# PathologyFoundation/plip

Measured on NVIDIA H100. Metric: image-text pairs/sec (224x224, 77-tok), higher is better.
Workload: dtype bf16

## Files before the change

### plip_b200/csrc/attention.cu

```cuda
#include <cfloat>

#include "kernels.cuh"
#include "wgmma.cuh"

namespace plip {

namespace {

constexpr int kAttThreads = 256;
constexpr uint32_t kTileBytes = 128 * 64 * 2;
constexpr uint32_t kStageBytes = 3 * kTileBytes;
constexpr uint32_t kAttSmem = kStageBytes + 1024 + 64;

__device__ __forceinline__ float fast_exp2(float x) {
  float y;
  asm("ex2.approx.ftz.f32 %0, %1;" : "=f"(y) : "f"(x));
  return y;
}
constexpr float kLog2e = 1.4426950408889634f;


template <bool F16, int NK>
__device__ __forceinline__ void qk_scores(float (&s)[NK / 2], uint64_t qdesc, uint64_t kdesc) {
  wgmma_pin(s);
  wgmma_fence();
#pragma unroll
  for (int k = 0; k < kHeadDim / 16; ++k) {
    if constexpr (NK == 64) wgmma_ss_n64<F16>(s, qdesc + 2 * k, kdesc + 2 * k, k != 0 ? 1u : 0u);
    else wgmma_ss_n128<F16>(s, qdesc + 2 * k, kdesc + 2 * k, k != 0 ? 1u : 0u);
  }
  wgmma_commit();
  wgmma_wait<0>();
  wgmma_pin(s);
}

__device__ __forceinline__ void quad_max(float& a, float& b) {
#pragma unroll
  for (int o = 1; o < 4; o <<= 1) {
    a = fmaxf(a, __shfl_xor_sync(0xffffffffu, a, o));
    b = fmaxf(b, __shfl_xor_sync(0xffffffffu, b, o));
  }
}
__device__ __forceinline__ void quad_sum(float& a, float& b) {
#pragma unroll
  for (int o = 1; o < 4; o <<= 1) {
    a += __shfl_xor_sync(0xffffffffu, a, o);
    b += __shfl_xor_sync(0xffffffffu, b, o);
  }
}

__device__ __forceinline__ int last_visible_key(int row, int S, int causal) {
  return row < S ? (causal ? row : S - 1) : -1;
}

template <int N>
__device__ __forceinline__ void mask_column(float (&s)[N], int j, int e, bool ok, int key, int lim0, int lim1) {
  if (!(ok && key <= lim0)) s[4 * j + e] = -INFINITY;
  if (!(ok && key <= lim1)) s[4 * j + 2 + e] = -INFINITY;
}

__device__ __forceinline__ float row_shift(float m) { return fmaxf(m * kLog2e, -FLT_MAX); }
__device__ __forceinline__ float row_inv(float l) { return l > 0.f ? 1.0f / l : 0.f; }

__device__ __forceinline__ float softmax_exp(float s, float ms) { return fast_exp2(fmaf(s, kLog2e, -ms)); }

__device__ __forceinline__ float2 fold_row_max(const float (&s)[32], float& m0, float& m1, float& l0, float& l1) {
  float mx0 = m0, mx1 = m1;
#pragma unroll
  for (int j = 0; j < 8; ++j) {
    mx0 = fmaxf(mx0, fmaxf(s[4 * j + 0], s[4 * j + 1]));
    mx1 = fmaxf(mx1, fmaxf(s[4 * j + 2], s[4 * j + 3]));
  }
  quad_max(mx0, mx1);
  const float alpha0 = softmax_exp(m0, row_shift(mx0)), alpha1 = softmax_exp(m1, row_shift(mx1));
  m0 = mx0;
  m1 = mx1;
  l0 *= alpha0;
  l1 *= alpha1;
  return make_float2(alpha0, alpha1);
}

template <bool F16, int N>
__device__ __forceinline__ void exp_sum_pack(const float (&s)[N], float ms0, float ms1, float& l0, float& l1,
                                             uint32_t (&pa)[N / 8][4]) {
#pragma unroll
  for (int j = 0; j < N / 4; ++j) {
    const float e00 = softmax_exp(s[4 * j + 0], ms0), e01 = softmax_exp(s[4 * j + 1], ms0);
    const float e10 = softmax_exp(s[4 * j + 2], ms1), e11 = softmax_exp(s[4 * j + 3], ms1);
    l0 += e00 + e01;
    l1 += e10 + e11;
    pa[j >> 1][2 * (j & 1) + 0] = pack_op2<F16>(e00, e01);
    pa[j >> 1][2 * (j & 1) + 1] = pack_op2<F16>(e10, e11);
  }
}

template <bool F16>
__device__ __forceinline__ void stage_rows(uint32_t row0, const float (&o)[32], float inv0, float inv1, int rr, int q4) {
  const uint32_t row1 = row0 + 8u * 128u;
#pragma unroll
  for (int j = 0; j < 8; ++j) {
    st_shared_b32(row0 + ((j ^ rr) << 4) + q4 * 4, pack_op2<F16>(o[4 * j + 0] * inv0, o[4 * j + 1] * inv0));
    st_shared_b32(row1 + ((j ^ rr) << 4) + q4 * 4, pack_op2<F16>(o[4 * j + 2] * inv1, o[4 * j + 3] * inv1));
  }
}

struct AttParams {
  int64_t n_seq;
  int seq_len;
  int slot;
  int group;
  int heads;
  int64_t seq_tiles;
  int causal;
  const int32_t* key_mask;
};

template <bool F16, int NK>
__global__ void __launch_bounds__(kAttThreads, NK == 64 ? 3 : 2)
attention_kernel(const __grid_constant__ CUtensorMap tmLoad, const __grid_constant__ CUtensorMap tmStore,
                 const AttParams p) {
  extern __shared__ uint8_t smem_raw[];
  const uint32_t smem_base = (smem_u32(smem_raw) + 1023u) & ~1023u;
  const uint32_t bar = smem_base + kStageBytes;
  const uint32_t sq = smem_base, sk = smem_base + kTileBytes, sv = smem_base + 2 * kTileBytes;

  const int warp = threadIdx.x >> 5;
  const int lane = threadIdx.x & 31;
  const int hf = warp >> 2;
  const int D = p.heads * kHeadDim;
  const int S = p.seq_len, G = p.group, slot = p.slot;

  if (threadIdx.x == 0) {
    tma_prefetch_desc(&tmLoad);
    tma_prefetch_desc(&tmStore);
    mbar_init(bar, 1);
    fence_mbar_init();
  }
  __syncthreads();

  const int ntiles = (int)(p.seq_tiles * p.heads);
  const uint32_t slot_bytes = static_cast<uint32_t>(slot) * 128u;
  auto issue_loads = [&](int tile) {
    const int64_t st = tile / p.heads;
    const int h = (int)(tile - st * p.heads);
    mbar_arrive_expect_tx(bar, 3 * kTileBytes);
    for (int g = 0; g < G; ++g) {
      const int32_t row = (int32_t)((st * G + g) * S);
      tma_load_2d(sq + g * slot_bytes, &tmLoad, bar, h * kHeadDim, row);
      tma_load_2d(sk + g * slot_bytes, &tmLoad, bar, D + h * kHeadDim, row);
      tma_load_2d(sv + g * slot_bytes, &tmLoad, bar, 2 * D + h * kHeadDim, row);
    }
  };
  if (threadIdx.x == 0 && (int)blockIdx.x < ntiles) issue_loads(blockIdx.x);

  const int q4 = lane & 3, rr = lane >> 2;
  const int R0 = 64 * hf + 16 * (warp & 3) + rr;
  const int g = R0 / slot;
  const int r_in0 = R0 - g * slot, r_in1 = r_in0 + 8;
  const int kbase = (NK == 64) ? 64 * hf : 0;
  const int k_in_base = kbase - g * slot + 2 * q4;
  const int lim0 = last_visible_key(r_in0, S, p.causal), lim1 = last_visible_key(r_in1, S, p.causal);

  uint32_t it = 0;
  for (int tile = blockIdx.x; tile < ntiles; tile += gridDim.x, ++it) {
    const int st = tile / p.heads;
    const int h = tile - st * p.heads;
    const int64_t seq = (int64_t)st * G + g;

    uint32_t kv = 0;
#pragma unroll
    for (int c = 0; c < NK / 4; ++c) {
      const int k_in = k_in_base + 8 * (c >> 1) + (c & 1);
      bool ok = k_in >= 0 && k_in < S;
      if (ok && p.key_mask != nullptr) ok = seq < p.n_seq && p.key_mask[seq * S + k_in] != 0;
      kv |= (ok ? 1u : 0u) << c;
    }

    mbar_wait(bar, it & 1u);

    float s[NK / 2];
    qk_scores<F16, NK>(s, make_smem_desc_sw128(sq + hf * (64 * 128), 1024, 16),
                       make_smem_desc_sw128(sk + kbase * 128, 1024, 16));

    float mx0 = -INFINITY, mx1 = -INFINITY;
#pragma unroll
    for (int c = 0; c < NK / 4; ++c) {
      const int j = c >> 1, e = c & 1;
      mask_column(s, j, e, (kv >> c) & 1u, k_in_base + 8 * j + e, lim0, lim1);
      mx0 = fmaxf(mx0, s[4 * j + e]);
      mx1 = fmaxf(mx1, s[4 * j + 2 + e]);
    }
    quad_max(mx0, mx1);
    float sum0 = 0.f, sum1 = 0.f;
    uint32_t pa[NK / 16][4];
    exp_sum_pack<F16>(s, row_shift(mx0), row_shift(mx1), sum0, sum1, pa);
    quad_sum(sum0, sum1);

    float o[32];
    wgmma_pin(o);
    wgmma_fence();
#pragma unroll
    for (int kk = 0; kk < NK / 16; ++kk) {
      const uint64_t vdesc = make_smem_desc_sw128(sv + (kbase + 16 * kk) * 128, 1024, 1024);
      wgmma_rs_n64<F16>(o, pa[kk], vdesc, kk != 0 ? 1u : 0u);
    }
    wgmma_commit();
    wgmma_wait<0>();
    wgmma_pin(o);

    stage_rows<F16>(sq + static_cast<uint32_t>(R0) * 128u, o, row_inv(sum0), row_inv(sum1), rr, q4);
    fence_proxy_async_smem();
    __syncthreads();
    if (threadIdx.x == 0) {
      for (int gg = 0; gg < G; ++gg) {
        const int64_t sq_idx = (int64_t)st * G + gg;
        if (sq_idx < p.n_seq)
          tma_store_2d(&tmStore, sq + static_cast<uint32_t>(gg * slot) * 128u, h * kHeadDim, (int32_t)(sq_idx * S));
      }
      tma_store_commit();
      tma_store_wait_read();
      if (tile + (int)gridDim.x < ntiles) issue_loads(tile + gridDim.x);
    }
  }
  if (threadIdx.x == 0) tma_store_wait_all();
}

template <bool F16, int NK>
int launch_attention_inst(const CUtensorMap& tmL, const CUtensorMap& tmS, const AttParams& p, cudaStream_t st) {
  auto kern = attention_kernel<F16, NK>;
  static unsigned long long configured = 0;
  static int grid_cap = 0;
  if (first_use_on_device(configured)) {
    PLIP_CUDA_CHECK(cudaFuncSetAttribute(kern, cudaFuncAttributeMaxDynamicSharedMemorySize, (int)kAttSmem));
    int dev = 0, sms = 0, per_sm = 0;
    PLIP_CUDA_CHECK(cudaGetDevice(&dev));
    PLIP_CUDA_CHECK(cudaDeviceGetAttribute(&sms, cudaDevAttrMultiProcessorCount, dev));
    PLIP_CUDA_CHECK(cudaOccupancyMaxActiveBlocksPerMultiprocessor(&per_sm, kern, kAttThreads, kAttSmem));
    grid_cap = (per_sm > 0 ? per_sm : 1) * sms;
  }
  const int64_t tiles = p.seq_tiles * p.heads;
  const int grid = (int)(tiles < grid_cap ? tiles : grid_cap);
  PLIP_CUDA_CHECK(launch_kernel(kern, dim3(grid), dim3(kAttThreads), kAttSmem, st, 1, tmL, tmS, p));
  return 0;
}

constexpr int kLongThreads = 288;
constexpr int kLongKeys = 64;
constexpr uint32_t kLongQBytes = 128 * 64 * 2;
constexpr uint32_t kLongKVBytes = kLongKeys * 64 * 2;
constexpr int kLongStages = 2;
constexpr uint32_t kLongSmem = kLongQBytes + kLongStages * 2 * kLongKVBytes + 1024 + 64;

struct LongAttParams {
  int seq_len;
  int heads;
  int q_blocks;
};

template <bool F16>
__global__ void __launch_bounds__(kLongThreads, 2)
attention_long_kernel(const __grid_constant__ CUtensorMap tmQKV, const __grid_constant__ CUtensorMap tmO,
                      const LongAttParams p) {
  extern __shared__ uint8_t smem_raw[];
  const uint32_t smem_base = (smem_u32(smem_raw) + 1023u) & ~1023u;
  const uint32_t sq = smem_base;
  auto sk = [&](int s) { return smem_base + kLongQBytes + (uint32_t)s * 2u * kLongKVBytes; };
  auto sv = [&](int s) { return sk(s) + kLongKVBytes; };
  const uint32_t bar = smem_base + kLongQBytes + kLongStages * 2 * kLongKVBytes;
  const uint32_t q_bar = bar;
  auto full_bar = [&](int s) { return bar + 8u * (1 + s); };
  auto empty_bar = [&](int s) { return bar + 8u * (1 + kLongStages + s); };

  const int warp = threadIdx.x >> 5;
  const int lane = threadIdx.x & 31;
  const int wg = warp >> 2;
  const int S = p.seq_len, D = p.heads * kHeadDim;
  const int qb = blockIdx.x % p.q_blocks;
  const int bh = blockIdx.x / p.q_blocks;
  const int h = bh % p.heads;
  const int seq = bh / p.heads;
  const int q0 = qb * 128;
  const int n_kb = (S + kLongKeys - 1) / kLongKeys;

  if (threadIdx.x == 0) {
    tma_prefetch_desc(&tmQKV);
    tma_prefetch_desc(&tmO);
    mbar_init(q_bar, 1);
    for (int s = 0; s < kLongStages; ++s) {
      mbar_init(full_bar(s), 1);
      mbar_init(empty_bar(s), 2);
    }
    fence_mbar_init();
  }
  __syncthreads();

  if (wg == 2) {
    if (lane == 0) {
      mbar_arrive_expect_tx(q_bar, kLongQBytes);
      tma_load_3d(sq, &tmQKV, q_bar, h * kHeadDim, q0, seq);
      tma_load_3d(sq + kLongQBytes / 2, &tmQKV, q_bar, h * kHeadDim, q0 + 64, seq);
      for (int kb = 0; kb < n_kb; ++kb) {
        const int s = kb % kLongStages;
        if (kb >= kLongStages) mbar_wait(empty_bar(s), (uint32_t)((kb / kLongStages - 1) & 1));
        mbar_arrive_expect_tx(full_bar(s), 2 * kLongKVBytes);
        tma_load_3d(sk(s), &tmQKV, full_bar(s), D + h * kHeadDim, kb * kLongKeys, seq);
        tma_load_3d(sv(s), &tmQKV, full_bar(s), 2 * D + h * kHeadDim, kb * kLongKeys, seq);
      }
    }
    return;
  }

  const int q4 = lane & 3, rr = lane >> 2;
  const int R0 = 64 * wg + 16 * (warp & 3) + rr;
  float o[32];
#pragma unroll
  for (int i = 0; i < 32; ++i) o[i] = 0.f;
  float m0 = -INFINITY, m1 = -INFINITY;
  float l0 = 0.f, l1 = 0.f;
  const uint64_t qdesc = make_smem_desc_sw128(sq + wg * (64 * 128), 1024, 16);
  mbar_wait(q_bar, 0);

  for (int kb = 0; kb < n_kb; ++kb) {
    const int s = kb % kLongStages;
    mbar_wait(full_bar(s), (uint32_t)((kb / kLongStages) & 1));

    float sc[32];
    qk_scores<F16, 64>(sc, qdesc, make_smem_desc_sw128(sk(s), 1024, 16));

    const int kbase = kb * kLongKeys + 2 * q4;
    if (kb * kLongKeys + kLongKeys > S) {
#pragma unroll
      for (int j = 0; j < 8; ++j)
#pragma unroll
        for (int e = 0; e < 2; ++e)
          if (kbase + 8 * j + e >= S) {
            sc[4 * j + e] = -INFINITY;
            sc[4 * j + 2 + e] = -INFINITY;
          }
    }
    const float2 alpha = fold_row_max(sc, m0, m1, l0, l1);
#pragma unroll
    for (int j = 0; j < 8; ++j) {
      o[4 * j + 0] *= alpha.x; o[4 * j + 1] *= alpha.x;
      o[4 * j + 2] *= alpha.y; o[4 * j + 3] *= alpha.y;
    }
    uint32_t pa[4][4];
    exp_sum_pack<F16>(sc, row_shift(m0), row_shift(m1), l0, l1, pa);

    wgmma_pin(o);
    wgmma_fence();
#pragma unroll
    for (int kk = 0; kk < kLongKeys / 16; ++kk) {
      const uint64_t vdesc = make_smem_desc_sw128(sv(s) + 16 * kk * 128, 1024, 1024);
      wgmma_rs_n64<F16>(o, pa[kk], vdesc, 1u);
    }
    wgmma_commit();
    wgmma_wait<0>();
    wgmma_pin(o);
    if ((threadIdx.x & 127) == 0) mbar_arrive(empty_bar(s));
  }

  quad_sum(l0, l1);
  stage_rows<F16>(sq + static_cast<uint32_t>(R0) * 128u, o, row_inv(l0), row_inv(l1), rr, q4);
  fence_proxy_async_smem();
  if (wg == 0) named_barrier_sync<1, 128>();
  else named_barrier_sync<2, 128>();
  if ((threadIdx.x & 127) == 0 && q0 + 64 * wg < S) {
    tma_store_3d(&tmO, sq + wg * (64 * 128), h * kHeadDim, q0 + 64 * wg, seq);
    tma_store_commit();
    tma_store_wait_all();
  }
}

constexpr int kProbThreads = 128;
constexpr int kProbStages = 2;
constexpr int kProbLd = 72;
constexpr uint32_t kProbTileBytes = 64 * 64 * 2;
constexpr uint32_t kProbStageOff = kProbTileBytes;
constexpr uint32_t kProbStagingOff = kProbStageOff + kProbStages * kProbTileBytes;
constexpr uint32_t kProbBarOff = kProbStagingOff + 64 * kProbLd * 4;
constexpr uint32_t kProbSmem = kProbBarOff + 8 * (1 + kProbStages) + 1024;

struct ProbParams {
  int seq_len;
  int heads;
  int q_blocks;
  int causal;
  const int32_t* key_mask;
  float* probs;
};

template <bool F16>
__global__ void __launch_bounds__(kProbThreads)
attention_probs_kernel(const __grid_constant__ CUtensorMap tmQKV, const ProbParams p) {
  extern __shared__ uint8_t smem_raw[];
  const uint32_t smem_base = (smem_u32(smem_raw) + 1023u) & ~1023u;
  float* staging = reinterpret_cast<float*>(smem_raw + (smem_base - smem_u32(smem_raw)) + kProbStagingOff);
  const uint32_t sq = smem_base;
  auto sk = [&](int s) { return smem_base + kProbStageOff + (uint32_t)s * kProbTileBytes; };
  const uint32_t q_bar = smem_base + kProbBarOff;
  auto full_bar = [&](int s) { return q_bar + 8u * (1 + s); };

  const int warp = threadIdx.x >> 5;
  const int lane = threadIdx.x & 31;
  const int S = p.seq_len, D = p.heads * kHeadDim;
  const int qb = blockIdx.x % p.q_blocks;
  const int64_t bh = blockIdx.x / p.q_blocks;
  const int h = (int)(bh % p.heads);
  const int64_t seq = bh / p.heads;
  const int q0 = qb * 64;
  const int n_kb = (S + 63) / 64;
  const bool resident = n_kb <= kProbStages;
  const int n_loads = resident ? n_kb : 2 * n_kb;

  auto issue_k = [&](int i) {
    const int s = i % kProbStages;
    mbar_arrive_expect_tx(full_bar(s), kProbTileBytes);
    tma_load_3d(sk(s), &tmQKV, full_bar(s), D + h * kHeadDim, (i % n_kb) * 64, (int32_t)seq);
  };
  if (threadIdx.x == 0) {
    tma_prefetch_desc(&tmQKV);
    mbar_init(q_bar, 1);
    for (int s = 0; s < kProbStages; ++s) mbar_init(full_bar(s), 1);
    fence_mbar_init();
    mbar_arrive_expect_tx(q_bar, kProbTileBytes);
    tma_load_3d(sq, &tmQKV, q_bar, h * kHeadDim, q0, (int32_t)seq);
    for (int i = 0; i < kProbStages && i < n_loads; ++i) issue_k(i);
  }
  __syncthreads();

  const int q4 = lane & 3, rr = lane >> 2;
  const int r0 = 16 * warp + rr;
  const int qa = q0 + r0, qc = qa + 8;
  const int lim0 = last_visible_key(qa, S, p.causal), lim1 = last_visible_key(qc, S, p.causal);
  const int32_t* km = p.key_mask ? p.key_mask + seq * S : nullptr;
  const uint64_t qdesc = make_smem_desc_sw128(sq, 1024, 16);
  mbar_wait(q_bar, 0);

  float sc[32];
  auto scores = [&](int u) {
    const int li = resident ? u % n_kb : u;
    const int s = li % kProbStages;
    mbar_wait(full_bar(s), (uint32_t)((li / kProbStages) & 1));
    qk_scores<F16, 64>(sc, qdesc, make_smem_desc_sw128(sk(s), 1024, 16));
    if (!resident) {
      __syncthreads();
      if (threadIdx.x == 0 && li + kProbStages < n_loads) issue_k(li + kProbStages);
    }
    const int kbase = (u % n_kb) * 64 + 2 * q4;
#pragma unroll
    for (int j = 0; j < 8; ++j)
#pragma unroll
      for (int e = 0; e < 2; ++e) {
        const int key = kbase + 8 * j + e;
        mask_column(sc, j, e, key < S && (km == nullptr || km[key] != 0), key, lim0, lim1);
      }
  };

  float m0 = -INFINITY, m1 = -INFINITY, l0 = 0.f, l1 = 0.f;
  for (int kb = 0; kb < n_kb; ++kb) {
    scores(kb);
    fold_row_max(sc, m0, m1, l0, l1);
    const float ms0 = row_shift(m0), ms1 = row_shift(m1);
#pragma unroll
    for (int j = 0; j < 8; ++j) {
      l0 += softmax_exp(sc[4 * j + 0], ms0) + softmax_exp(sc[4 * j + 1], ms0);
      l1 += softmax_exp(sc[4 * j + 2], ms1) + softmax_exp(sc[4 * j + 3], ms1);
    }
  }
  quad_sum(l0, l1);
  const float ms0 = row_shift(m0), ms1 = row_shift(m1);
  const float inv0 = row_inv(l0), inv1 = row_inv(l1);

  float* wst = staging + 16 * warp * kProbLd;
  const int rows = S - (q0 + 16 * warp) < 16 ? S - (q0 + 16 * warp) : 16;
  float* out_base = p.probs + ((seq * p.heads + h) * (int64_t)S + q0 + 16 * warp) * S;
  for (int kb = 0; kb < n_kb; ++kb) {
    scores(n_kb + kb);
#pragma unroll
    for (int j = 0; j < 8; ++j) {
      *reinterpret_cast<float2*>(wst + rr * kProbLd + 8 * j + 2 * q4) =
          make_float2(softmax_exp(sc[4 * j + 0], ms0) * inv0, softmax_exp(sc[4 * j + 1], ms0) * inv0);
      *reinterpret_cast<float2*>(wst + (rr + 8) * kProbLd + 8 * j + 2 * q4) =
          make_float2(softmax_exp(sc[4 * j + 2], ms1) * inv1, softmax_exp(sc[4 * j + 3], ms1) * inv1);
    }
    __syncwarp();
    const int k0 = kb * 64;
    const int nc = S - k0 < 64 ? S - k0 : 64;
    const int total = rows > 0 ? rows * nc : 0;
    int r = 0, c = lane;
    while (c >= nc) { c -= nc; ++r; }
    for (int i = lane; i < total; i += 32) {
      __stcs(out_base + (int64_t)r * S + k0 + c, wst[r * kProbLd + c]);
      c += 32;
      while (c >= nc) { c -= nc; ++r; }
    }
    __syncwarp();
  }
}

template <auto Kern, int Threads, uint32_t Smem, typename... Args>
int launch_blocks(int64_t blocks, cudaStream_t st, const Args&... args) {
  static unsigned long long configured = 0;
  if (first_use_on_device(configured))
    PLIP_CUDA_CHECK(cudaFuncSetAttribute(Kern, cudaFuncAttributeMaxDynamicSharedMemorySize, (int)Smem));
  PLIP_CUDA_CHECK(launch_kernel(Kern, dim3((unsigned)blocks), dim3(Threads), Smem, st, 1, args...));
  return 0;
}

int check_attention_args(const char* fn, const void* qkv, const void* out, int64_t n_seq, int seq_len, int heads) {
  PLIP_REQUIRE(qkv && out, "%s: null argument", fn);
  PLIP_REQUIRE(n_seq > 0 && seq_len > 0 && seq_len <= kMaxVisSeq, "%s: bad shape n_seq=%lld seq_len=%d", fn,
               (long long)n_seq, seq_len);
  PLIP_REQUIRE(heads > 0 && heads <= 16, "%s: bad head count %d", fn, heads);
  return 0;
}

int make_seq_tmap(CUtensorMap* tm, const void* base, int64_t n_seq, int seq_len, int cols) {
  return make_tmap_bf16_3d(tm, base, (uint64_t)n_seq, (uint64_t)seq_len, (uint64_t)cols, (uint64_t)cols * 2,
                           (uint64_t)seq_len * cols * 2, 64, 64);
}

}

int launch_attention(const __nv_bfloat16* qkv, int64_t n_seq, int seq_len, int heads, bool causal,
                     const int32_t* key_mask, __nv_bfloat16* out, int f16, cudaStream_t st) {
  if (int rc = check_attention_args("attention", qkv, out, n_seq, seq_len, heads)) return rc;
  const int D = heads * kHeadDim;
  if (seq_len > 128) {
    PLIP_REQUIRE(!causal && key_mask == nullptr,
                 "attention: seq_len %d > 128 is supported without causal or key mask only", seq_len);
    LongAttParams p;
    p.seq_len = seq_len;
    p.heads = heads;
    p.q_blocks = (seq_len + 127) / 128;
    const int64_t blocks = n_seq * heads * p.q_blocks;
    PLIP_REQUIRE(blocks < 0x7fffffff && n_seq < 0x7fffffff, "attention: too many sequences");
    CUtensorMap tmQKV, tmO;
    if (int rc = make_seq_tmap(&tmQKV, qkv, n_seq, seq_len, 3 * D)) return rc;
    if (int rc = make_seq_tmap(&tmO, out, n_seq, seq_len, D)) return rc;
    return f16 ? launch_blocks<attention_long_kernel<true>, kLongThreads, kLongSmem>(blocks, st, tmQKV, tmO, p)
               : launch_blocks<attention_long_kernel<false>, kLongThreads, kLongSmem>(blocks, st, tmQKV, tmO, p);
  }
  const int64_t rows = n_seq * seq_len;
  PLIP_REQUIRE(rows + 128 < 0x7fffffff, "attention: too many token rows");
  AttParams p;
  p.n_seq = n_seq;
  p.seq_len = seq_len;
  p.slot = seq_len <= 32 ? 32 : (seq_len <= 64 ? 64 : 128);
  p.group = 128 / p.slot;
  p.heads = heads;
  p.seq_tiles = (n_seq + p.group - 1) / p.group;
  p.causal = causal ? 1 : 0;
  p.key_mask = key_mask;
  CUtensorMap tmL, tmS;
  if (int rc = make_tmap_bf16_2d(&tmL, qkv, (uint64_t)rows, (uint64_t)3 * D, (uint64_t)3 * D * 2, (uint32_t)p.slot, 64)) return rc;
  if (int rc = make_tmap_bf16_2d(&tmS, out, (uint64_t)rows, (uint64_t)D, (uint64_t)D * 2, (uint32_t)seq_len, 64)) return rc;
  PLIP_REQUIRE(p.seq_tiles * heads < 0x7fffffff, "attention: too many tiles");
  if (p.slot == 128) return f16 ? launch_attention_inst<true, 128>(tmL, tmS, p, st) : launch_attention_inst<false, 128>(tmL, tmS, p, st);
  return f16 ? launch_attention_inst<true, 64>(tmL, tmS, p, st) : launch_attention_inst<false, 64>(tmL, tmS, p, st);
}

int launch_attention_probs(const __nv_bfloat16* qkv, int64_t n_seq, int seq_len, int heads, bool causal,
                           const int32_t* key_mask, float* probs, int f16, cudaStream_t st) {
  if (int rc = check_attention_args("attention_probs", qkv, probs, n_seq, seq_len, heads)) return rc;
  ProbParams p;
  p.seq_len = seq_len;
  p.heads = heads;
  p.q_blocks = (seq_len + 63) / 64;
  p.causal = causal ? 1 : 0;
  p.key_mask = key_mask;
  p.probs = probs;
  const int64_t blocks = n_seq * heads * p.q_blocks;
  PLIP_REQUIRE(blocks < 0x7fffffff && n_seq < 0x7fffffff, "attention_probs: too many sequences");
  const int D = heads * kHeadDim;
  CUtensorMap tm;
  if (int rc = make_seq_tmap(&tm, qkv, n_seq, seq_len, 3 * D)) return rc;
  return f16 ? launch_blocks<attention_probs_kernel<true>, kProbThreads, kProbSmem>(blocks, st, tm, p)
             : launch_blocks<attention_probs_kernel<false>, kProbThreads, kProbSmem>(blocks, st, tm, p);
}

}
```

Measured before the change: 26970.

## Double-buffer attention tiles, skip dead rows, shorten causal chains, use 3D TMA loads

For the 128-key variant the attention kernel now keeps two shared-memory stages with separate mbarriers, so the loads for the next tile overlap compute on the current one. Warps whose rows fall past the sequence length skip the softmax and the output staging. Under a causal mask, the first warpgroup runs only 64 keys instead of 128. Q/K/V loads switch to a 3D tensor map indexed per sequence, so rows past a short sequence are zero-filled rather than read from the next sequence. In exchange, the NK=128 path uses double the shared memory, which may reduce occupancy, and the code adds a branchy helper template.

```diff
diff --git a/plip_b200/csrc/attention.cu b/plip_b200/csrc/attention.cu
--- a/plip_b200/csrc/attention.cu
+++ b/plip_b200/csrc/attention.cu
@@ -10,7 +10,6 @@
 constexpr int kAttThreads = 256;
 constexpr uint32_t kTileBytes = 128 * 64 * 2;
 constexpr uint32_t kStageBytes = 3 * kTileBytes;
-constexpr uint32_t kAttSmem = kStageBytes + 1024 + 64;
 
 __device__ __forceinline__ float fast_exp2(float x) {
   float y;
@@ -115,14 +114,58 @@
   const int32_t* key_mask;
 };
 
+template <bool F16, int NKW>
+__device__ __forceinline__ void attend_rows(uint32_t sq, uint32_t sk, uint32_t sv, int hf, int kbase, int k_in_base,
+                                            uint32_t kv, int lim0, int lim1, bool live, int R0, int rr, int q4) {
+  float s[NKW / 2];
+  qk_scores<F16, NKW>(s, make_smem_desc_sw128(sq + hf * (64 * 128), 1024, 16),
+                      make_smem_desc_sw128(sk + kbase * 128, 1024, 16));
+
+  float sum0 = 0.f, sum1 = 0.f;
+  uint32_t pa[NKW / 16][4] = {};
+  if (live) {
+    float mx0 = -INFINITY, mx1 = -INFINITY;
+#pragma unroll
+    for (int c = 0; c < NKW / 4; ++c) {
+      const int j = c >> 1, e = c & 1;
+      mask_column(s, j, e, (kv >> c) & 1u, k_in_base + 8 * j + e, lim0, lim1);
+      mx0 = fmaxf(mx0, s[4 * j + e]);
+      mx1 = fmaxf(mx1, s[4 * j + 2 + e]);
+    }
+    quad_max(mx0, mx1);
+    exp_sum_pack<F16>(s, row_shift(mx0), row_shift(mx1), sum0, sum1, pa);
+    quad_sum(sum0, sum1);
+  }
+
+  float o[32];
+  wgmma_pin(o);
+  wgmma_fence();
+#pragma unroll
+  for (int kk = 0; kk < NKW / 16; ++kk) {
+    const uint64_t vdesc = make_smem_desc_sw128(sv + (kbase + 16 * kk) * 128, 1024, 1024);
+    wgmma_rs_n64<F16>(o, pa[kk], vdesc, kk != 0 ? 1u : 0u);
+  }
+  wgmma_commit();
+  wgmma_wait<0>();
+  wgmma_pin(o);
+
+  if (live) stage_rows<F16>(sq + static_cast<uint32_t>(R0) * 128u, o, row_inv(sum0), row_inv(sum1), rr, q4);
+}
+
+template <int NK>
+constexpr int kAttStages = NK == 128 ? 2 : 1;
+template <int NK>
+constexpr uint32_t kAttSmem = kAttStages<NK> * kStageBytes + 1024 + 64;
+
 template <bool F16, int NK>
 __global__ void __launch_bounds__(kAttThreads, NK == 64 ? 3 : 2)
 attention_kernel(const __grid_constant__ CUtensorMap tmLoad, const __grid_constant__ CUtensorMap tmStore,
                  const AttParams p) {
+  constexpr int kStages = kAttStages<NK>;
   extern __shared__ uint8_t smem_raw[];
   const uint32_t smem_base = (smem_u32(smem_raw) + 1023u) & ~1023u;
-  const uint32_t bar = smem_base + kStageBytes;
-  const uint32_t sq = smem_base, sk = smem_base + kTileBytes, sv = smem_base + 2 * kTileBytes;
+  const uint32_t bar0 = smem_base + kStages * kStageBytes;
+  auto sq = [&](int s) { return smem_base + (uint32_t)s * kStageBytes; };
 
   const int warp = threadIdx.x >> 5;
   const int lane = threadIdx.x & 31;
@@ -133,39 +176,46 @@
   if (threadIdx.x == 0) {
     tma_prefetch_desc(&tmLoad);
     tma_prefetch_desc(&tmStore);
-    mbar_init(bar, 1);
+    for (int s = 0; s < kStages; ++s) mbar_init(bar0 + 8u * s, 1);
     fence_mbar_init();
   }
   __syncthreads();
 
   const int ntiles = (int)(p.seq_tiles * p.heads);
   const uint32_t slot_bytes = static_cast<uint32_t>(slot) * 128u;
-  auto issue_loads = [&](int tile) {
+  auto issue_loads = [&](int tile, int s) {
     const int64_t st = tile / p.heads;
     const int h = (int)(tile - st * p.heads);
+    const uint32_t bar = bar0 + 8u * s;
     mbar_arrive_expect_tx(bar, 3 * kTileBytes);
     for (int g = 0; g < G; ++g) {
-      const int32_t row = (int32_t)((st * G + g) * S);
-      tma_load_2d(sq + g * slot_bytes, &tmLoad, bar, h * kHeadDim, row);
-      tma_load_2d(sk + g * slot_bytes, &tmLoad, bar, D + h * kHeadDim, row);
-      tma_load_2d(sv + g * slot_bytes, &tmLoad, bar, 2 * D + h * kHeadDim, row);
+      const int32_t seq = (int32_t)(st * G + g);
+      const uint32_t dst = sq(s) + g * slot_bytes;
+      tma_load_3d(dst, &tmLoad, bar, h * kHeadDim, 0, seq);
+      tma_load_3d(dst + kTileBytes, &tmLoad, bar, D + h * kHeadDim, 0, seq);
+      tma_load_3d(dst + 2 * kTileBytes, &tmLoad, bar, 2 * D + h * kHeadDim, 0, seq);
     }
   };
-  if (threadIdx.x == 0 && (int)blockIdx.x < ntiles) issue_loads(blockIdx.x);
+  if (threadIdx.x == 0)
+    for (int s = 0; s < kStages; ++s)
+      if ((int)blockIdx.x + s * (int)gridDim.x < ntiles) issue_loads(blockIdx.x + s * gridDim.x, s);
 
   const int q4 = lane & 3, rr = lane >> 2;
   const int R0 = 64 * hf + 16 * (warp & 3) + rr;
   const int g = R0 / slot;
   const int r_in0 = R0 - g * slot, r_in1 = r_in0 + 8;
+  const bool live = r_in0 - rr < S;
   const int kbase = (NK == 64) ? 64 * hf : 0;
   const int k_in_base = kbase - g * slot + 2 * q4;
   const int lim0 = last_visible_key(r_in0, S, p.causal), lim1 = last_visible_key(r_in1, S, p.causal);
+  const bool short_chain = NK == 128 && p.causal && hf == 0;
 
   uint32_t it = 0;
   for (int tile = blockIdx.x; tile < ntiles; tile += gridDim.x, ++it) {
     const int st = tile / p.heads;
     const int h = tile - st * p.heads;
     const int64_t seq = (int64_t)st * G + g;
+    const int s = (int)(it % kStages);
 
     uint32_t kv = 0;
 #pragma unroll
@@ -176,50 +226,24 @@
       kv |= (ok ? 1u : 0u) << c;
     }
 
-    mbar_wait(bar, it & 1u);
-
-    float s[NK / 2];
-    qk_scores<F16, NK>(s, make_smem_desc_sw128(sq + hf * (64 * 128), 1024, 16),
-                       make_smem_desc_sw128(sk + kbase * 128, 1024, 16));
-
-    float mx0 = -INFINITY, mx1 = -INFINITY;
-#pragma unroll
-    for (int c = 0; c < NK / 4; ++c) {
-      const int j = c >> 1, e = c & 1;
-      mask_column(s, j, e, (kv >> c) & 1u, k_in_base + 8 * j + e, lim0, lim1);
-      mx0 = fmaxf(mx0, s[4 * j + e]);
-      mx1 = fmaxf(mx1, s[4 * j + 2 + e]);
-    }
-    quad_max(mx0, mx1);
-    float sum0 = 0.f, sum1 = 0.f;
-    uint32_t pa[NK / 16][4];
-    exp_sum_pack<F16>(s, row_shift(mx0), row_shift(mx1), sum0, sum1, pa);
-    quad_sum(sum0, sum1);
-
-    float o[32];
-    wgmma_pin(o);
-    wgmma_fence();
-#pragma unroll
-    for (int kk = 0; kk < NK / 16; ++kk) {
-      const uint64_t vdesc = make_smem_desc_sw128(sv + (kbase + 16 * kk) * 128, 1024, 1024);
-      wgmma_rs_n64<F16>(o, pa[kk], vdesc, kk != 0 ? 1u : 0u);
-    }
-    wgmma_commit();
-    wgmma_wait<0>();
-    wgmma_pin(o);
-
-    stage_rows<F16>(sq + static_cast<uint32_t>(R0) * 128u, o, row_inv(sum0), row_inv(sum1), rr, q4);
+    mbar_wait(bar0 + 8u * s, (it / kStages) & 1u);
+
+    const uint32_t sk = sq(s) + kTileBytes, sv = sq(s) + 2 * kTileBytes;
+    if (short_chain) attend_rows<F16, 64>(sq(s), sk, sv, hf, kbase, k_in_base, kv, lim0, lim1, live, R0, rr, q4);
+    else attend_rows<F16, NK>(sq(s), sk, sv, hf, kbase, k_in_base, kv, lim0, lim1, live, R0, rr, q4);
+
     fence_proxy_async_smem();
     __syncthreads();
     if (threadIdx.x == 0) {
       for (int gg = 0; gg < G; ++gg) {
         const int64_t sq_idx = (int64_t)st * G + gg;
         if (sq_idx < p.n_seq)
-          tma_store_2d(&tmStore, sq + static_cast<uint32_t>(gg * slot) * 128u, h * kHeadDim, (int32_t)(sq_idx * S));
+          tma_store_2d(&tmStore, sq(s) + static_cast<uint32_t>(gg * slot) * 128u, h * kHeadDim, (int32_t)(sq_idx * S));
       }
       tma_store_commit();
       tma_store_wait_read();
-      if (tile + (int)gridDim.x < ntiles) issue_loads(tile + gridDim.x);
+      const int next = tile + kStages * (int)gridDim.x;
+      if (next < ntiles) issue_loads(next, s);
     }
   }
   if (threadIdx.x == 0) tma_store_wait_all();
@@ -228,19 +252,20 @@
 template <bool F16, int NK>
 int launch_attention_inst(const CUtensorMap& tmL, const CUtensorMap& tmS, const AttParams& p, cudaStream_t st) {
   auto kern = attention_kernel<F16, NK>;
+  constexpr uint32_t smem = kAttSmem<NK>;
   static unsigned long long configured = 0;
   static int grid_cap = 0;
   if (first_use_on_device(configured)) {
-    PLIP_CUDA_CHECK(cudaFuncSetAttribute(kern, cudaFuncAttributeMaxDynamicSharedMemorySize, (int)kAttSmem));
+    PLIP_CUDA_CHECK(cudaFuncSetAttribute(kern, cudaFuncAttributeMaxDynamicSharedMemorySize, (int)smem));
     int dev = 0, sms = 0, per_sm = 0;
     PLIP_CUDA_CHECK(cudaGetDevice(&dev));
     PLIP_CUDA_CHECK(cudaDeviceGetAttribute(&sms, cudaDevAttrMultiProcessorCount, dev));
-    PLIP_CUDA_CHECK(cudaOccupancyMaxActiveBlocksPerMultiprocessor(&per_sm, kern, kAttThreads, kAttSmem));
+    PLIP_CUDA_CHECK(cudaOccupancyMaxActiveBlocksPerMultiprocessor(&per_sm, kern, kAttThreads, smem));
     grid_cap = (per_sm > 0 ? per_sm : 1) * sms;
   }
   const int64_t tiles = p.seq_tiles * p.heads;
   const int grid = (int)(tiles < grid_cap ? tiles : grid_cap);
-  PLIP_CUDA_CHECK(launch_kernel(kern, dim3(grid), dim3(kAttThreads), kAttSmem, st, 1, tmL, tmS, p));
+  PLIP_CUDA_CHECK(launch_kernel(kern, dim3(grid), dim3(kAttThreads), smem, st, 1, tmL, tmS, p));
   return 0;
 }
 
@@ -554,7 +579,8 @@
   p.causal = causal ? 1 : 0;
   p.key_mask = key_mask;
   CUtensorMap tmL, tmS;
-  if (int rc = make_tmap_bf16_2d(&tmL, qkv, (uint64_t)rows, (uint64_t)3 * D, (uint64_t)3 * D * 2, (uint32_t)p.slot, 64)) return rc;
+  if (int rc = make_tmap_bf16_3d(&tmL, qkv, (uint64_t)n_seq, (uint64_t)seq_len, (uint64_t)3 * D, (uint64_t)3 * D * 2,
+                                 (uint64_t)seq_len * 3 * D * 2, (uint32_t)p.slot, 64)) return rc;
   if (int rc = make_tmap_bf16_2d(&tmS, out, (uint64_t)rows, (uint64_t)D, (uint64_t)D * 2, (uint32_t)seq_len, 64)) return rc;
   PLIP_REQUIRE(p.seq_tiles * heads < 0x7fffffff, "attention: too many tiles");
   if (p.slot == 128) return f16 ? launch_attention_inst<true, 128>(tmL, tmS, p, st) : launch_attention_inst<false, 128>(tmL, tmS, p, st);
```

Result: faster. 27450, median of 6 (+1.8%).
